# AaronZ345/StyleSinger

Hardware: AMD Instinct MI355X
Metric: mel-frames/sec (end-to-end infer incl. vocoder) (higher is better)
Workload: dtype f32; 1 GPU; c2: batch=8x8.0s utterances per GPU (T=1500 frames, Tp=28, Tr=1500), 100 mel + 2x100 f0 diffusion steps + HiFi-GAN-NSF, exact fp32 MFMA; global_batch=8, frames_per_utterance=1500, parallelism=dp1, diffusion_loops=hipGraph replay, hipgraph_captures=6, frame_bucket=64, mfma_precision=fp32, step_overlap=3 HIP streams: consecutive batches run concurrently

## Files before the change

include/stylesinger_hip.h:

```cpp
#ifndef STYLESINGER_HIP_H
#define STYLESINGER_HIP_H

#include <stdint.h>

#ifdef __cplusplus
extern "C" {
#endif

#define SS_ABI_VERSION 20
#define SS_MAX_TAPS 16
#define SS_MAX_LAYERS 32

const char* ss_last_error(void);
int ss_abi_version(void);
int ss_device_info(int dev, int* n_cu, char* arch, int arch_len);
int ss_struct_sizes(int64_t* out, int n);
int ss_set_tuning(const char* key, int value);
int ss_get_tuning(const char* key);
int ss_set_clock_probe(void* dev_u64x2);
int ss_set_q4_guard(void* dev_u32x2);
int ss_debug_null_launch(int grid, int block, void* stream);

enum {
  SS_EPI_STORE = 0,
  SS_EPI_GATE = 1,
  SS_EPI_RESSKIP = 2,
  SS_EPI_DDPM = 3
};
enum { SS_ACT_NONE_ = 0, SS_ACT_RELU_ = 1, SS_ACT_GELU_ = 2, SS_ACT_MISH_ = 3, SS_ACT_TANH_ = 4, SS_ACT_LRELU_ = 5 };

enum { SS_TILE_AUTO = 0, SS_TILE_128x128 = 1, SS_TILE_64x128 = 2, SS_TILE_64x64 = 3, SS_TILE_128x64 = 4, SS_TILE_128x32 = 5 };

typedef struct ss_conv_gemm_args {
  const float* A;
  int64_t a_batch_stride;
  int32_t lda;
  int32_t Cin;
  int32_t ntaps;
  int32_t tap_off[SS_MAX_TAPS];
  const int32_t* lens;
  int32_t B, T;
  const float* a_bias;
  float a_scale;
  float a_lrelu;
  const float* W;
  int32_t N;
  int32_t Np;
  int32_t Kp;
  int32_t epi;
  const float* bias;
  float pre_scale;
  int32_t act;
  float act_slope;
  const float* E;
  int32_t lde;
  int64_t e_batch_stride;
  int32_t gate_mode;
  const float* R;
  int32_t ldr;
  int64_t r_batch_stride;
  float post_scale;
  int32_t accumulate;
  int32_t mask_rows;
  float* C;
  int32_t ldc;
  int64_t c_batch_stride;
  float* C2;
  int32_t ldc2;
  int64_t c2_batch_stride;
  int32_t Nh;
  float ddpm_recip, ddpm_recipm1, ddpm_c1, ddpm_c2, ddpm_sigma;
  const float* noise;
  uint64_t seed;
  const uint64_t* seed_dev;
  uint32_t step;
  int32_t tile;
  int32_t group_size;
  int64_t w_group_stride, bias_group_stride, a_bias_group_stride;
  int32_t mfma_bf16;
  int32_t ddpm_x0_pred;
  int32_t e_tiled;
  int32_t reserved2_;
} ss_conv_gemm_args;

int ss_conv_gemm(const ss_conv_gemm_args* args, void* stream);

int ss_gemm16_res(const ss_conv_gemm_args* args, int mt, void* stream);
int ss_gemm16_pick(int B, int T, int N);
int ss_gemm16_store(const ss_conv_gemm_args* args, int mt, void* stream);
int ss_gemm16_store_splitk(const ss_conv_gemm_args* args, int mt, int ksplit, float* partials, void* stream);
int ss_gemm16_ksplit_pick(int B, int T, int N, int K);

int ss_gemm16_resw(const ss_conv_gemm_args* args, const float* W16, int mt, void* stream);
int ss_pack_gemm16_weights(const float* src, float* dst, int Np, int Kp, void* stream);
int ss_wino43_gate16w(const ss_conv_gemm_args* args, const float* W16, int dilation, int mt, void* stream);
int ss_pack_gate16_weights(const float* src, float* dst, int Np, int Kp, void* stream);
int ss_wino43_gate16x(const ss_conv_gemm_args* args, const void* Wx, int dilation, int mt, void* stream);
int ss_split3_weights(const float* src, void* dst, int Np, int Kp, void* stream);
int ss_gemm16x_store(const ss_conv_gemm_args* args, const void* Wx, int mt, void* stream);
int ss_split3_gemm16_weights(const float* src, void* dst, int Np, int Kp, void* stream);
int64_t ss_split3_gemm16_elems(int Np, int Kp);
int ss_wino43_conv(const ss_conv_gemm_args* args, int k, int dilation, void* stream);
int ss_wino43_conv_ok(int C, int k, int dilation);
int ss_wino43_conv_ok4(int Cin, int Cout, int k, int dilation);
int ss_wino_gate(const ss_conv_gemm_args* args, int dilation, void* stream);
int ss_wino_weight_transform(const float* src, float* dst, int Cout, int Cin, void* stream);
int ss_wino43_gate(const ss_conv_gemm_args* args, int dilation, void* stream);
int ss_wino43_gate16(const ss_conv_gemm_args* args, int dilation, int mt, void* stream);
int ss_gate16_tile_addend(const float* E, int lde, int64_t e_batch_stride, float* E16, int B, int T, int Np, int dilation, int mt, void* stream);
int64_t ss_gate16_tiled_floats(int B, int T, int Np, int dilation, int mt);
int ss_wino43_gate16_pick(int B, int T, int Np, int dilation);
int ss_wino43_weight_transform(const float* src, float* dst, int Cout, int Cin, void* stream);

enum {
  SS_HEPI_STORE = 0,
  SS_HEPI_GATE = 1,
  SS_HEPI_RESX = 2
};
typedef struct ss_gemm_bf16_args {
  const uint16_t* A;
  int64_t a_batch_stride;
  int32_t lda;
  int32_t K;
  int32_t ntaps;
  int32_t tap_off[4];
  const int32_t* lens;
  int32_t B, T;
  const uint16_t* W;
  int64_t w_group_stride;
  int32_t N, Np;
  int32_t epi;
  int32_t act;
  const float* bias;
  int64_t bias_group_stride;
  const float* E;
  int32_t lde;
  int32_t gate_mode;
  int64_t e_batch_stride;
  float* X;
  int64_t x_batch_stride;
  int32_t ldx;
  float post_scale;
  const float* next_bias;
  int64_t next_bias_group_stride;
  uint16_t* Y;
  int64_t y_batch_stride;
  int32_t ldy;
  int32_t ldc;
  void* C;
  int64_t c_batch_stride;
  int32_t mask_rows;
  int32_t group_size;
  int32_t split;
  float out_scale;
  float q_scale;
  int32_t one_product;
  const float* cur_bias;
  int64_t cur_bias_group_stride;
  int32_t a_compact;
  int32_t reserved2_;
} ss_gemm_bf16_args;
int ss_gemm_bf16(const ss_gemm_bf16_args* args, void* stream);
int ss_gemm_bf16_gate256(const ss_gemm_bf16_args* args, void* stream);
int ss_gemm_bf16_gate256_ok(const ss_gemm_bf16_args* args);
int ss_gemm_bf16_gate128(const ss_gemm_bf16_args* args, void* stream);
int ss_gemm_bf16_gate128_ok(const ss_gemm_bf16_args* args);
int ss_gemm_bf16_gate128q(const ss_gemm_bf16_args* args, void* stream);
int ss_gemm_bf16_gate128q_ok(const ss_gemm_bf16_args* args);
int ss_gate128q_kindex(int32_t* out, int n);
int ss_gemm_bf16_tile256q(const ss_gemm_bf16_args* args, void* stream);
int ss_gemm_bf16_tile256q_ok(const ss_gemm_bf16_args* args);
int ss_tile256q_kindex(int32_t* out, int n_pairs);
int ss_gemm_bf16_tile256(const ss_gemm_bf16_args* args, void* stream);
int ss_gemm_bf16_tile256_ok(const ss_gemm_bf16_args* args);
typedef struct ss_layer512_args {
  const uint16_t* Hin;
  int32_t d;
  int32_t n_products;
  uint16_t* Hout;
  void* P;
  const int32_t* lens;
  int32_t B, T;
  const uint16_t* Wg;
  const uint16_t* Wr;
  const float* E512;
  uint16_t* G;
  int64_t g_batch_stride;
// ... 305 lines not shown
```

stylesinger_amd/csrc/hifigan.hip:

```cpp
#include "common.h"
#include "../../include/stylesinger_hip.h"

namespace {

constexpr int NH = 9;
constexpr int HOP_MAX = 1024;
constexpr size_t LDS_MAX = 160 * 1024;

inline int64_t align_up(int64_t x, int64_t a) { return (x + a - 1) / a * a; }
inline int round_up32(int x) { return (x + 31) / 32 * 32; }

struct HgWs {
  int32_t* lens;
  double* base;
  double* q;
  float* r0;
  float* har;
  float* pre;
  float* x;
  float* xs;
  float* ta;
  float* tb;
  int64_t bytes;
};
// ... 257 lines not shown
__global__ __launch_bounds__(256) void conv_post_kernel(const float* __restrict__ x, const float* __restrict__ w,
                                                        const float* __restrict__ bias, float* __restrict__ wav,
                                                        const int32_t* __restrict__ lens, int B, int64_t L, int C, int k) {
  extern __shared__ float smem[];
  const int ldx = C + 1;
  float* xs = smem;
  float* wsh = smem + (256 + k - 1) * ldx;
  const int tiles = (int)((L + 255) / 256);
  const int b = blockIdx.x / tiles;
  const int64_t i0 = (int64_t)(blockIdx.x % tiles) * 256;
  const int tid = threadIdx.x;
  const int64_t valid = lens ? (int64_t)lens[b] : L;
  const int half = (k - 1) / 2;
  for (int i = tid; i < k * C; i += 256) {
    const int j = i / C, c = i % C;
    wsh[i] = w[c * k + j];
  }
  const int rows = 256 + k - 1;
  for (int i = tid; i < rows * C; i += 256) {
    const int r = i / C, c = i % C;
    const int64_t idx = i0 - half + r;
    float v = 0.f;
    if (idx >= 0 && idx < valid && idx < L) {
      v = x[((int64_t)b * L + idx) * C + c];
      v = v >= 0.f ? v : v * 0.01f;
    }
    xs[r * ldx + c] = v;
  }
  __syncthreads();
  const int64_t i = i0 + tid;
  if (i >= L) return;
  float acc = bias[0];
  for (int j = 0; j < k; ++j)
    for (int c = 0; c < C; ++c) acc += wsh[j * C + c] * xs[(tid + j) * ldx + c];
  wav[(int64_t)b * L + i] = (i < valid) ? tanhf(acc) : 0.f;
}

inline ss_conv_gemm_args base_args(int B, int T, const int32_t* lens) {
  ss_conv_gemm_args a;
  memset(&a, 0, sizeof(a));
  a.B = B;
  a.T = T;
  a.lens = lens;
  a.ntaps = 1;
  a.a_scale = 1.0f;
  a.a_lrelu = 1.0f;
  a.pre_scale = 1.0f;
  a.post_scale = 1.0f;
  a.mask_rows = 1;
  return a;
}

int conv_same(const float* A, int B, int Trows, int C, const int32_t* lens, const float* W, const float* W_wino, const float* bias, int k,
              int d, float lrelu, int act_out, const float* R, float post_scale, int accumulate, float* out, int bf16, hipStream_t stream) {
  ss_conv_gemm_args a = base_args(B, Trows, lens);
  a.mfma_bf16 = bf16;
  a.A = A;
  a.lda = C;
  a.a_batch_stride = (int64_t)Trows * C;
  a.Cin = C;
  a.ntaps = k;
  for (int j = 0; j < k; ++j) a.tap_off[j] = (j - (k - 1) / 2) * d;
  a.a_lrelu = lrelu;
  a.W = W;
  a.N = C;
  a.Np = round_up32(C);
  a.Kp = round_up32(C);
  a.epi = SS_EPI_STORE;
  a.bias = bias;
  a.R = R;
  a.ldr = C;
  a.r_batch_stride = (int64_t)Trows * C;
  a.post_scale = post_scale;
  a.accumulate = accumulate;
  a.C = out;
  a.ldc = C;
  a.c_batch_stride = (int64_t)Trows * C;
  if (act_out) {
    a.act = SS_ACT_LRELU_;
    a.act_slope = 0.1f;
  }
  if (W_wino && ((int64_t)Trows + 1024) * C * 4 < ((int64_t)g_ss_tuning.voc_wino_max_mb << 20)) {
    a.W = W_wino;
    return ss_wino43_conv(&a, k, d, stream);
  }
  return ss_conv_gemm(&a, stream);
}

}

extern "C" int64_t ss_hifigan_workspace_bytes(const ss_hifigan* hg, int B, int T) {
  if (!hg || B <= 0 || T <= 0) return -1;
  return hg_layout(hg, B, T, nullptr).bytes;
}

extern "C" int ss_hifigan_source(const ss_hifigan* hg, const float* f0, int B, int T, const float* rand_ini,
                                 const float* sine_noise, uint64_t seed, float* har, void* ws, int64_t ws_bytes,
                                 void* stream_) {
  hipStream_t stream = (hipStream_t)stream_;
  SS_CHECK_ARG(hg && f0 && har && ws, "ss_hifigan_source: null pointer");
  SS_CHECK_ARG(hg->harmonics + 1 == NH, "ss_hifigan_source: harmonic_num must be 8");
  const int hop = hop_of(hg);
  SS_CHECK_ARG(hop % 64 == 0 && hop <= HOP_MAX, "ss_hifigan_source: hop=%d must be a multiple of 64 and <= %d", hop, HOP_MAX);
  const HgWs w = hg_layout(hg, B, T, ws);
  SS_CHECK_ARG(ws_bytes >= w.bytes, "ss_hifigan_source: workspace too small");
  const float sr = (float)hg->sr;
  hipLaunchKernelGGL(src_base_kernel, dim3(B * NH), dim3(256), 0, stream, f0, rand_ini, seed, w.base, w.r0, B, T, hop, sr);
  SS_CHECK_LAUNCH("src_base_kernel");
  hipLaunchKernelGGL(src_frame_sum_kernel, dim3(B * T), dim3(hop), 0, stream, f0, w.base, w.r0, w.q, B, T, hop, sr);
  SS_CHECK_LAUNCH("src_frame_sum_kernel");
  hipLaunchKernelGGL(src_scan_kernel, dim3(B * NH), dim3(256), 0, stream, w.q, B * NH, T);
  SS_CHECK_LAUNCH("src_scan_kernel");
  hipLaunchKernelGGL(src_final_kernel, dim3(B * T), dim3(hop), 0, stream, f0, w.base, w.r0, w.q, sine_noise, seed,
                     hg->src_w, hg->src_b, har, B, T, hop, sr);
  SS_CHECK_LAUNCH("src_final_kernel");
  return SS_OK;
}

extern "C" int ss_hifigan_forward(const ss_hifigan* hg, const float* mel, const float* f0, const int32_t* lens, int B, int T,
                                  const float* rand_ini, const float* sine_noise, uint64_t seed, float* wav,
                                  float* har_source_out, void* ws, int64_t ws_bytes, void* stream_) {
  hipStream_t stream = (hipStream_t)stream_;
  SS_CHECK_ARG(hg && mel && f0 && wav && ws, "ss_hifigan_forward: null pointer");
  SS_CHECK_ARG(hg->n_ups >= 1 && hg->n_ups <= SS_HG_MAX_UPS && hg->n_kernels >= 1 && hg->n_kernels <= SS_HG_MAX_KERNELS,
               "ss_hifigan_forward: bad config");
  const HgWs w = hg_layout(hg, B, T, ws);
  SS_CHECK_ARG(ws_bytes >= w.bytes, "ss_hifigan_forward: workspace too small (%lld < %lld)", (long long)ws_bytes, (long long)w.bytes);
  const int hop = hop_of(hg);
  const int64_t L = (int64_t)T * hop;

  hipLaunchKernelGGL(stage_lens_kernel, dim3((B + 63) / 64), dim3(64), 0, stream, lens, w.lens, B, T, hg->n_ups,
                     hg->up_rate[0], hg->up_rate[1], hg->up_rate[2], hg->up_rate[3], hg->up_rate[4], hg->up_rate[5]);
  SS_CHECK_LAUNCH("stage_lens_kernel");

  float* har = har_source_out ? har_source_out : w.har;
  SS_PROPAGATE(ss_hifigan_source(hg, f0, B, T, rand_ini, sine_noise, seed, har, ws, ws_bytes, stream_));

  {
    ss_conv_gemm_args a = base_args(B, T, w.lens);
    a.A = mel;
    a.lda = 80;
    a.a_batch_stride = (int64_t)T * 80;
    a.Cin = 80;
    a.ntaps = 7;
    for (int j = 0; j < 7; ++j) a.tap_off[j] = j - 3;
    a.W = hg->w_pre;
    a.N = hg->c0;
    a.Np = round_up32(hg->c0);
    a.Kp = 96;
    a.epi = SS_EPI_STORE;
    a.bias = hg->b_pre;
    a.C = w.pre;
    a.ldc = hg->c0;
    a.c_batch_stride = (int64_t)T * hg->c0;
    a.mfma_bf16 = hg->mfma_bf16;
    SS_PROPAGATE(ss_conv_gemm(&a, stream));
  }

  const float* cur = w.pre;
  int rows_in = T, cin = hg->c0, R = 1;
  for (int i = 0; i < hg->n_ups; ++i) {
    const int u = hg->up_rate[i], ku = hg->up_k[i];
    const int cout = hg->c0 >> (i + 1);
    const int pad = (ku - u) / 2;
    const int nph0 = u - pad;
    const int rows_out = rows_in * u;
// ... 80 lines not shown
```

stylesinger_amd/lib.py:

```python
import ctypes as C
import os

import torch

from . import abi
from .abi import declarations, declared_symbols

HERE = os.path.dirname(os.path.abspath(__file__))
LIB_PATH = os.environ.get("SS_LIB_PATH") or os.path.join(HERE, "libstylesinger_hip.so")

SS_MAX_TAPS, SS_MAX_LAYERS, SS_HG_MAX_UPS, SS_HG_MAX_KERNELS = (abi.DEFINES[n] for n in ("SS_MAX_TAPS", "SS_MAX_LAYERS", "SS_HG_MAX_UPS", "SS_HG_MAX_KERNELS"))
ABI_VERSION = abi.DEFINES["SS_ABI_VERSION"]
ALIGN_MAX_T, ALIGN_MAX_LC = abi.DEFINES["SS_ALIGN_MAX_T"], abi.DEFINES["SS_ALIGN_MAX_LC"]
EPI_STORE, EPI_GATE, EPI_RESSKIP, EPI_DDPM = (abi.ENUMS["SS_EPI_" + n] for n in ("STORE", "GATE", "RESSKIP", "DDPM"))
ACT_NONE, ACT_RELU, ACT_GELU, ACT_MISH, ACT_TANH, ACT_LRELU = (abi.ENUMS[f"SS_ACT_{n}_"] for n in ("NONE", "RELU", "GELU", "MISH", "TANH", "LRELU"))
HEPI_STORE, HEPI_GATE, HEPI_RESX = (abi.ENUMS["SS_HEPI_" + n] for n in ("STORE", "GATE", "RESX"))

_STRUCT_SIZES_ORDER = ("ss_conv_gemm_args", "ss_wavenet", "ss_hifigan", "ss_gemm_bf16_args", "ss_f0track_params", "ss_layer512_args")
ConvGemmArgs, WaveNet, HifiGan, GemmBf16Args, F0TrackParams, Layer512Args = (abi.STRUCTURES[n] for n in _STRUCT_SIZES_ORDER)


class StyleSingerHipError(RuntimeError):
    pass

# ... 93 lines not shown


def gate16_tile_addend(E, *, B, T, Np, lde, e_bs, dilation, mt):
    n = load().ss_gate16_tiled_floats(B, T, Np, int(dilation), int(mt))
    out = torch.empty(n, device=E.device, dtype=torch.float32)
    check(load().ss_gate16_tile_addend(ptr(E), lde, e_bs, ptr(out), B, T, Np, int(dilation), int(mt), stream_ptr()), "ss_gate16_tile_addend")
    return out


def wino_gate(A, Wt, out, *, dilation, **kw):
    kw.setdefault("epi", EPI_GATE)
    a = _fill_args(A, Wt, out, **kw)
    check(load().ss_wino_gate(C.byref(a), int(dilation), stream_ptr()), "ss_wino_gate")


def wino43_gate(A, Wt, out, *, dilation, **kw):
    kw.setdefault("epi", EPI_GATE)
    a = _fill_args(A, Wt, out, **kw)
    check(load().ss_wino43_gate(C.byref(a), int(dilation), stream_ptr()), "ss_wino43_gate")


def pack_gemm16_weights(Wp, Kp):
    Wp = Wp.contiguous().float()
    out = torch.empty_like(Wp)
    check(load().ss_pack_gemm16_weights(ptr(Wp), ptr(out), Wp.shape[0], Kp, stream_ptr()), "ss_pack_gemm16_weights")
    return out


def pack_gate16_weights(Wp, Kp):
    Wp = Wp.contiguous().float()
    out = torch.empty_like(Wp)
    check(load().ss_pack_gate16_weights(ptr(Wp), ptr(out), Wp.shape[0], Kp, stream_ptr()), "ss_pack_gate16_weights")
    return out


def wino43_gate16(A, Wt, out, *, dilation, mt=0, W16=None, **kw):
    kw.setdefault("epi", EPI_GATE)
    a = _fill_args(A, Wt, out, **kw)
    if W16 is not None:
        check(load().ss_wino43_gate16w(C.byref(a), ptr(W16), int(dilation), int(mt), stream_ptr()), "ss_wino43_gate16w")
        return
    check(load().ss_wino43_gate16(C.byref(a), int(dilation), int(mt), stream_ptr()), "ss_wino43_gate16")


def gemm16_res(A, W, out, *, mt=0, W16=None, **kw):
    a = _fill_args(A, W, out, **kw)
    if W16 is not None:
        check(load().ss_gemm16_resw(C.byref(a), ptr(W16), int(mt), stream_ptr()), "ss_gemm16_resw")
        return
    check(load().ss_gemm16_res(C.byref(a), int(mt), stream_ptr()), "ss_gemm16_res")


def gemm16_store(A, W, out, *, mt=0, **kw):
    a = _fill_args(A, W, out, **kw)
    check(load().ss_gemm16_store(C.byref(a), int(mt), stream_ptr()), "ss_gemm16_store")


def gemm16_store_splitk(A, W, out, *, ksplit, mt=0, **kw):
    a = _fill_args(A, W, out, **kw)
    part = torch.empty(max(1, ksplit) * a.B * a.T * a.N, device=out.device, dtype=torch.float32)
    check(load().ss_gemm16_store_splitk(C.byref(a), int(mt), int(ksplit), ptr(part), stream_ptr()), "ss_gemm16_store_splitk")


def wino43_weight(w):
    w = w.contiguous().float()
    out = torch.empty(w.shape[0], w.shape[1], 6, device=w.device, dtype=torch.float32)
    check(load().ss_wino43_weight_transform(ptr(w), ptr(out), w.shape[0], w.shape[1], stream_ptr()), "ss_wino43_weight_transform")
    return out


def wino43_group_weight(w):
    w = w.contiguous().float()
    Cout, Cin, k = w.shape
    G = (k + 2) // 3
    wp = torch.zeros(Cout, Cin, 3 * G, device=w.device, dtype=torch.float32)
    wp[..., :k] = w
    return torch.cat([wino43_weight(wp[..., 3 * g:3 * g + 3]) for g in range(G)], dim=-1).contiguous()


def wino43_conv(A, W, out, *, k, dilation, **kw):
    taps = [(j - (k - 1) // 2) * dilation for j in range(k)]
    a = _fill_args(A, W, out, taps=taps, **kw)
    check(load().ss_wino43_conv(C.byref(a), k, dilation, stream_ptr()), "ss_wino43_conv")
    return out


def split3_weights(Wp, Kp):
    Wp = Wp.contiguous().float()
    Np = Wp.shape[0]
    out = torch.empty(Np, 3 * Wp.shape[1], device=Wp.device, dtype=torch.bfloat16)
    check(load().ss_split3_weights(ptr(Wp), ptr(out), Np, Kp, stream_ptr()), "ss_split3_weights")
    return out


def split3_gemm16_weights(Wp, Kp):
    Wp = Wp.contiguous().float()
    Np = Wp.shape[0]
    out = torch.empty(int(load().ss_split3_gemm16_elems(Np, Kp)), device=Wp.device, dtype=torch.bfloat16)
    check(load().ss_split3_gemm16_weights(ptr(Wp), ptr(out), Np, Kp, stream_ptr()), "ss_split3_gemm16_weights")
    return out


def gemm16x_store(A, W, Wx, out, *, mt=0, **kw):
    a = _fill_args(A, W, out, **kw)
    check(load().ss_gemm16x_store(C.byref(a), ptr(Wx), int(mt), stream_ptr()), "ss_gemm16x_store")


def wino43_gate16x(A, Wx, out, *, dilation, mt=0, **kw):
    kw.setdefault("epi", EPI_GATE)
    a = _fill_args(A, Wx, out, **kw)
    check(load().ss_wino43_gate16x(C.byref(a), ptr(Wx), dilation, mt, stream_ptr()), "ss_wino43_gate16x")
    return out


def wino_weight(w):
    w = w.contiguous().float()
    out = torch.empty(w.shape[0], w.shape[1], 4, device=w.device, dtype=torch.float32)
    check(load().ss_wino_weight_transform(ptr(w), ptr(out), w.shape[0], w.shape[1], stream_ptr()), "ss_wino_weight_transform")
    return out


def pack_conv_weight(w, *, scale0=None, interleave_half=0, row_scale=1.0):
    if w.dim() == 2:
        w = w[:, :, None]
    w = w.contiguous().float()
    Cout, Cin, k = w.shape
    Kp = round_up(Cin, 32)
    Np = 2 * round_up(interleave_half, 32) if interleave_half else round_up(Cout, 32)
    dst = torch.empty(Np, k * Kp, device=w.device, dtype=torch.float32)
    check(load().ss_pack_conv_weight(ptr(w), ptr(scale0), ptr(dst), Cout, Cin, k, Np, Kp, interleave_half, _f(row_scale),
                                     stream_ptr()), "ss_pack_conv_weight")
    return dst


def weight_norm_scale(v, g):
    v = v.contiguous().float()
    g = g.contiguous().float().reshape(-1)
    rows = v.shape[0]
    out = torch.empty(rows, device=v.device, dtype=torch.float32)
    check(load().ss_weight_norm_scale(ptr(v), ptr(g), ptr(out), rows, v.numel() // rows, stream_ptr()), "ss_weight_norm_scale")
    return out


def pack_convtr_weight(w, scale0, u, group):
    w = w.contiguous().float()
    Cin, Cout, k = w.shape
    pad = (k - u) // 2
    nph = (u - pad) if group == 0 else pad
    Np = round_up(nph * Cout, 32)
    Kp = round_up(Cin, 32)
    dst = torch.empty(Np, 2 * Kp, device=w.device, dtype=torch.float32)
    check(load().ss_pack_convtr_weight(ptr(w), ptr(scale0), ptr(dst), Cin, Cout, k, u, group, Np, Kp, stream_ptr()),
          "ss_pack_convtr_weight")
    return dst


def pack_bias(b, *, b2=None, Np=None, interleave_half=0, repeat=1):
    b = b.contiguous().float()
    n = b.numel()
    if Np is None:
        Np = 2 * round_up(interleave_half, 32) if interleave_half else round_up(n * repeat, 32)
    dst = torch.empty(Np, device=b.device, dtype=torch.float32)
    check(load().ss_pack_bias(ptr(b), ptr(b2), ptr(dst), n, Np, interleave_half, repeat, stream_ptr()), "ss_pack_bias")
    return dst


# ... 275 lines not shown
```

stylesinger_amd/vocoder.py:

```python
import ctypes

import numpy as np
import torch

from . import lib as L
from . import spec as _spec
from .config import make_hparams, make_vocoder_config
from .denoise import denoise_batch, geometry as denoise_geometry, resolve_denoise

REGISTERED_VOCODERS = {}


def register_vocoder(name):
    def _f(cls):
        REGISTERED_VOCODERS[name] = cls
        return cls
    return _f


def get_vocoder_cls(hparams):
    return REGISTERED_VOCODERS[hparams["vocoder"]]


CONV_POST_MAX_CHANNELS = 128
# ... 34 lines not shown
        bad("upsample_initial_channel", f"must halve {len(rates)} times into a multiple of 4 channels")
    if c0 >> len(rates) > CONV_POST_MAX_CHANNELS:
        bad("upsample_initial_channel", f"leaves {c0 >> len(rates)} channels for conv_post, at most {CONV_POST_MAX_CHANNELS}")
    rk, rd = cfg.get("resblock_kernel_sizes"), cfg.get("resblock_dilation_sizes")
    if not ints(rk) or not 1 <= len(rk) <= L.SS_HG_MAX_KERNELS:
        bad("resblock_kernel_sizes", f"1 to {L.SS_HG_MAX_KERNELS} integer kernel sizes")
    for k in rk:
        if k < 1 or k % 2 == 0 or k > L.SS_MAX_TAPS:
            bad("resblock_kernel_sizes", f"kernel {k}: odd and at most {L.SS_MAX_TAPS} taps")
    if not isinstance(rd, (list, tuple)) or len(rd) != len(rk):
        bad("resblock_dilation_sizes", "one list of dilations per ResBlock kernel size")
    for d in rd:
        if not ints(d) or len(d) != 3 or min(d) < 1:
            bad("resblock_dilation_sizes", f"{list(d) if isinstance(d, (list, tuple)) else d!r}: exactly three positive dilations per ResBlock")
    return cfg


class HifiGanGeneratorHIP(torch.nn.Module):

    def __init__(self, h=None):
        super().__init__()
        self.h = make_vocoder_config(h)
        self._names = []
        for name, shape in _spec.vocoder_spec(self.h):
            self._names.append(name)
            self.register_buffer("p__" + name.replace(".", "__"), torch.zeros(*shape))
        self._pk = None
        self._weights_version = 0
        self._packed_version = -1
        self.hop = int(np.prod(self.h["upsample_rates"]))

    def p(self, name):
        return getattr(self, "p__" + name.replace(".", "__"))

    def state_dict(self, *a, **k):
        return {n: self.p(n) for n in self._names}

    def load_state_dict(self, state_dict, strict=True):
        missing = [n for n in self._names if n not in state_dict]
        unexpected = [k for k in state_dict if k not in set(self._names)]
        if strict and (missing or unexpected):
            raise RuntimeError(f"HifiGanGeneratorHIP.load_state_dict: missing={missing[:5]} unexpected={unexpected[:5]}")
        with torch.no_grad():
            for n in self._names:
                if n in state_dict:
                    self.p(n).copy_(state_dict[n])
        self._weights_version += 1
        return torch.nn.modules.module._IncompatibleKeys(missing, unexpected)

    def remove_weight_norm(self):
        return self

    def _wn(self, prefix):
        v, g = self.p(prefix + ".weight_v"), self.p(prefix + ".weight_g")
        return v, L.weight_norm_scale(v, g)

    def pack(self):
        h = check_config(self.h)
        dev = self.p("conv_pre.bias").device
        if dev.type != "cuda":
            raise L.StyleSingerHipError("HifiGanGeneratorHIP needs its weights on a GPU: there is no CPU path")
        keep = []
        hg = L.HifiGan()
        rates, ks = h["upsample_rates"], h["upsample_kernel_sizes"]
        hg.n_ups, hg.n_kernels, hg.c0 = len(rates), len(h["resblock_kernel_sizes"]), h["upsample_initial_channel"]
        hg.sr, hg.harmonics = h["audio_sample_rate"], h["harmonic_num"]
        import os
        hg.mfma_bf16 = 1 if os.environ.get("SS_PRECISION", h.get("mfma_precision", "fp32")) == "bf16" else 0
        hg.wino = 1 if (not hg.mfma_bf16 and os.environ.get("SS_VOC_WINO", str(h.get("vocoder_wino", 1))) != "0") else 0
        lib = L.load()
        for i, (u, k) in enumerate(zip(rates, ks)):
            hg.up_rate[i], hg.up_k[i] = u, k
        for i in range(len(rates), L.SS_HG_MAX_UPS):
            hg.up_rate[i], hg.up_k[i] = 1, 1
        for j, k in enumerate(h["resblock_kernel_sizes"]):
            hg.rb_k[j] = k
            for m, d in enumerate(h["resblock_dilation_sizes"][j]):
                hg.rb_d[j][m] = d

        def hold(t):
            keep.append(t)
            return t.data_ptr()

        v, s0 = self._wn("conv_pre")
        hg.w_pre = hold(L.pack_conv_weight(v, scale0=s0))
        hg.b_pre = hold(L.pack_bias(self.p("conv_pre.bias")))
        nk = hg.n_kernels
        for i, u in enumerate(rates):
            v, s0 = self._wn(f"ups.{i}")
            for g in range(2):
                hg.w_up[i][g] = hold(L.pack_convtr_weight(v, s0, u, g))
            hg.b_up[i] = hold(L.pack_bias(self.p(f"ups.{i}.bias"), repeat=u))
            hg.w_noise[i] = hold(self.p(f"noise_convs.{i}.weight").contiguous())
            hg.b_noise[i] = hold(self.p(f"noise_convs.{i}.bias").contiguous())
            for j in range(nk):
                for m in range(3):
                    pfx = f"resblocks.{i * nk + j}"
                    k, d = h["resblock_kernel_sizes"][j], h["resblock_dilation_sizes"][j][m]
                    cout = hg.c0 >> (i + 1)
                    v, s0 = self._wn(f"{pfx}.convs1.{m}")
                    hg.w_rb1[i][j][m] = hold(L.pack_conv_weight(v, scale0=s0))
                    hg.b_rb1[i][j][m] = hold(L.pack_bias(self.p(f"{pfx}.convs1.{m}.bias")))
                    if hg.wino and lib.ss_wino43_conv_ok(cout, k, d):
                        hg.w_rb1_wino[i][j][m] = hold(L.pack_conv_weight(L.wino43_group_weight(v * s0.view(-1, 1, 1))))
                    v, s0 = self._wn(f"{pfx}.convs2.{m}")
                    hg.w_rb2[i][j][m] = hold(L.pack_conv_weight(v, scale0=s0))
                    hg.b_rb2[i][j][m] = hold(L.pack_bias(self.p(f"{pfx}.convs2.{m}.bias")))
                    if hg.wino and lib.ss_wino43_conv_ok(cout, k, 1):
                        hg.w_rb2_wino[i][j][m] = hold(L.pack_conv_weight(L.wino43_group_weight(v * s0.view(-1, 1, 1))))
        v, s0 = self._wn("conv_post")
        hg.w_post = hold((v * s0.view(-1, 1, 1)).contiguous())
        hg.b_post = hold(self.p("conv_post.bias").contiguous())
        hg.src_w = hold(self.p("m_source.l_linear.weight").reshape(-1).contiguous())
        hg.src_b = hold(self.p("m_source.l_linear.bias").contiguous())
        self._pk = dict(hg=hg, keep=keep)
        self._packed_version = self._weights_version
        self._pack_device = dev
        torch.cuda.synchronize()

    def _ensure_packed(self):
        dev = self.p("conv_pre.bias").device
        if self._pk is None or self._packed_version != self._weights_version or self._pack_device != dev:
            self.pack()

    @torch.no_grad()
    def forward(self, mel, f0, lens=None, noise=None, seed=1234, return_source=False):
        self._ensure_packed()
        lib = L.load()
        hg = self._pk["hg"]
        mel = mel.contiguous().float()
        f0 = f0.contiguous().float()
        B, T, _ = mel.shape
        dev = mel.device
        Ls = T * self.hop
        wav = torch.empty(B, Ls, device=dev, dtype=torch.float32)
        har = torch.empty(B, Ls, device=dev, dtype=torch.float32) if return_source else None
        ws_bytes = lib.ss_hifigan_workspace_bytes(ctypes.addressof(hg), B, T)
        ws = torch.empty(ws_bytes, device=dev, dtype=torch.uint8)
        ri = sn = None
        if noise is not None:
            ri = noise["rand_ini"].to(dev).contiguous().float()
            sn = noise["sine_noise"].to(dev).contiguous().float()
        L.check(lib.ss_hifigan_forward(ctypes.addressof(hg), L.ptr(mel), L.ptr(f0), L.ptr(lens), B, T, L.ptr(ri), L.ptr(sn), seed,
                                       L.ptr(wav), L.ptr(har), L.ptr(ws), ws_bytes, L.stream_ptr()), "ss_hifigan_forward")
        return (wav, har) if return_source else wav


class BaseVocoder:
    def spec2wav(self, mel, **kwargs):
        raise NotImplementedError


@register_vocoder("HifiGAN_NSF")
class HifiGAN(BaseVocoder):

    def __init__(self, config=None, state_dict=None, device="cuda", hparams=None):
        self.hparams = make_hparams(hparams)
        self._denoise_v = resolve_denoise(self.hparams)
        self.config = make_vocoder_config(config)
        self.device = torch.device(device)
        self.model = HifiGanGeneratorHIP(self.config)
        if state_dict is not None:
            self.model.load_state_dict(state_dict, strict=True)
        self.model.remove_weight_norm()
        self.model.eval().to(self.device)

    def spec2wav(self, mel, **kwargs):
        f0 = kwargs.get("f0")
        if f0 is None or not self.hparams.get("use_nsf", True):
            raise NotImplementedError("the HIP vocoder implements the NSF path (use_nsf: true, f0 given)")
        c = torch.as_tensor(np.asarray(mel), dtype=torch.float32)[None].to(self.device)
        f = torch.as_tensor(np.asarray(f0), dtype=torch.float32)[None].to(self.device)
        y = self.model(c, f, noise=kwargs.get("noise"), seed=kwargs.get("seed", 1234))
        if self._denoise_v is not None:
            n_fft, hop = denoise_geometry(self.hparams)
            y, _ = denoise_batch(y, [y.shape[1]], n_fft, hop, n_fft, self._denoise_v)
        return y.view(-1).cpu().numpy()

    def spec2wav_batch(self, mel, f0, lens=None, **kwargs):
        out = self.model(mel, f0, lens=lens, **kwargs)
        if self._denoise_v is None:
            return out
        n_fft, hop = denoise_geometry(self.hparams)
        if hop != self.model.hop:
            raise L.StyleSingerHipError(f"vocoder_denoise_c: hop_size={hop} is not supported on the batched path: must equal the generator's hop "
                                        f"({self.model.hop})")
        wav = out[0] if isinstance(out, tuple) else out
        wav, _ = denoise_batch(wav, None if lens is None else lens * hop, n_fft, hop, n_fft, self._denoise_v)
        return (wav,) + tuple(out[1:]) if isinstance(out, tuple) else wav
```

Baseline: 44280 mel-frames/s.

## Add Winograd F(4,4) conv kernel for vocoder resblocks with k=7/11

Adds a new Winograd F(4,4) 1D convolution kernel using 7 transformed points per group of 4 taps. The vocoder resblock convs dispatch to it whenever it needs fewer MFMA products than the existing F(4,3) path, which is the case for kernel sizes 7 and 11. The goal is to cut the multiply work in the HiFi-GAN resblocks. In exchange it uses larger input-transform coefficients (up to 5 and 32/45), which can cost fp32 accuracy, and it brings a new pipelined kernel with its own LDS double-buffering.

```diff
diff --git a/include/stylesinger_hip.h b/include/stylesinger_hip.h
--- a/include/stylesinger_hip.h
+++ b/include/stylesinger_hip.h
@@ -103,6 +103,8 @@
 int ss_wino43_conv(const ss_conv_gemm_args* args, int k, int dilation, void* stream);
 int ss_wino43_conv_ok(int C, int k, int dilation);
 int ss_wino43_conv_ok4(int Cin, int Cout, int k, int dilation);
+int ss_wino44_conv(const ss_conv_gemm_args* args, int k, int dilation, void* stream);
+int ss_wino44_conv_ok(int C, int k, int dilation);
 int ss_wino_gate(const ss_conv_gemm_args* args, int dilation, void* stream);
 int ss_wino_weight_transform(const float* src, float* dst, int Cout, int Cin, void* stream);
 int ss_wino43_gate(const ss_conv_gemm_args* args, int dilation, void* stream);
diff --git a/stylesinger_amd/csrc/hifigan.hip b/stylesinger_amd/csrc/hifigan.hip
--- a/stylesinger_amd/csrc/hifigan.hip
+++ b/stylesinger_amd/csrc/hifigan.hip
@@ -363,6 +363,7 @@
   }
   if (W_wino && ((int64_t)Trows + 1024) * C * 4 < ((int64_t)g_ss_tuning.voc_wino_max_mb << 20)) {
     a.W = W_wino;
+    if (ss_wino44_conv_ok(C, k, d)) return ss_wino44_conv(&a, k, d, stream);
     return ss_wino43_conv(&a, k, d, stream);
   }
   return ss_conv_gemm(&a, stream);
diff --git a/stylesinger_amd/csrc/wino44_conv.hip b/stylesinger_amd/csrc/wino44_conv.hip
--- /dev/null
+++ b/stylesinger_amd/csrc/wino44_conv.hip
@@ -0,0 +1,373 @@
+#include "common.h"
+#include "device_prims.h"
+#include "../../include/stylesinger_hip.h"
+#include <type_traits>
+
+namespace {
+
+using namespace ss_dev;
+
+constexpr int BK = 32;
+constexpr int LD = BK;
+constexpr int BQ = 64;
+constexpr int NC = 7;
+constexpr int NR = 7;
+
+template <int D>
+__device__ __forceinline__ int frame_of_quad(int q) {
+  if constexpr (D == 1) return 4 * q;
+  else return (q / D) * (4 * D) + (q % D);
+}
+
+template <int D, bool LRELU, int BN>
+__global__ __launch_bounds__(BN * 4, BN == 64 ? 2 : 1) void wino44_conv_kernel(const ss_conv_gemm_args a, int q_tiles_per_item, int q_tiles,
+                                                                               int n_tiles, int groups, int lo_rows) {
+  static_assert(BN == 64 || BN == 32, "column tile of 64 or 32");
+  constexpr int NT = BN * 4;
+  constexpr int RP = NT / 8;
+  constexpr int AP = BQ / RP;
+  constexpr int BP = BN / RP;
+  extern __shared__ __attribute__((aligned(16))) float smem[];
+  float* As = smem;
+  float* Bs = smem + 2 * BQ * LD;
+
+  const int id = blockIdx.x;
+  const int grp = id / (8 * n_tiles);
+  const int rem = id % (8 * n_tiles);
+  const int qt = grp * 8 + (rem & 7);
+  const int nt = rem >> 3;
+  if (qt >= q_tiles) return;
+  const int b = __builtin_amdgcn_readfirstlane(qt / q_tiles_per_item);
+  const int q0 = __builtin_amdgcn_readfirstlane((qt % q_tiles_per_item) * BQ);
+  const int n0 = nt * BN;
+
+  const int tid = threadIdx.x, lane = tid & 63, wave = tid >> 6;
+  const int wm = BN == 64 ? wave >> 1 : wave, wn = BN == 64 ? wave & 1 : 0;
+  const int l31 = lane & 31, lh = lane >> 5;
+
+  const int len = ss_uniform_len(a.lens, b, a.T);
+  const int kchunks = a.Kp / BK;
+  const int ldw = groups * NC * a.Kp;
+
+  const __amdgpu_buffer_rsrc_t rsrc_a = __builtin_amdgcn_make_buffer_rsrc(
+      uniform_ptr(a.A + (int64_t)b * a.a_batch_stride), 0, __builtin_amdgcn_readfirstlane(len * a.lda * 4), 0x00020000);
+  const __amdgpu_buffer_rsrc_t rsrc_w =
+      __builtin_amdgcn_make_buffer_rsrc(uniform_ptr(a.W), 0, __builtin_amdgcn_readfirstlane(a.Np * ldw * 4), 0x00020000);
+
+  const int st_c4 = tid & 7;
+  const int st_row = tid >> 3;
+  int roff[AP];
+#pragma unroll
+  for (int i = 0; i < AP; ++i) roff[i] = ((frame_of_quad<D>(q0 + st_row + i * RP) - lo_rows) * a.lda + st_c4 * 4) * 4;
+  const int row_step = D * a.lda * 4;
+  const int group_step = 4 * row_step;
+  int w_voff[BP];
+#pragma unroll
+  for (int i = 0; i < BP; ++i) w_voff[i] = ((n0 + st_row + i * RP) * ldw + st_c4 * 4) * 4;
+
+  using Yes = std::true_type;
+  using No = std::false_type;
+  u32x4 rr[AP][NR], rb[BP];
+  auto load_rows = [&](int ci0b, auto ends) {
+    ci0b = __builtin_amdgcn_readfirstlane(ci0b);
+#pragma unroll
+    for (int i = 0; i < AP; ++i)
+#pragma unroll
+      for (int r = 0; r < NR; ++r)
+        if ((r == 0 || r == NR - 1) == decltype(ends)::value) rr[i][r] = __builtin_amdgcn_raw_buffer_load_b128(rsrc_a, roff[i] + r * row_step, ci0b, 0);
+  };
+  auto load_b = [&](int cb) {
+    cb = __builtin_amdgcn_readfirstlane(cb);
+#pragma unroll
+    for (int i = 0; i < BP; ++i) rb[i] = __builtin_amdgcn_raw_buffer_load_b128(rsrc_w, w_voff[i], cb, 0);
+  };
+  const float slope = a.a_lrelu;
+  auto act_rows = [&]() {
+    if constexpr (LRELU) {
+#pragma unroll
+      for (int i = 0; i < AP; ++i)
+#pragma unroll
+        for (int r = 0; r < NR; ++r) {
+          const f32x4 v = __builtin_bit_cast(f32x4, rr[i][r]);
+          const f32x4 sv = v * slope;
+          f32x4 o;
+          o.x = ss_lrelu_max(v.x, sv.x);
+          o.y = ss_lrelu_max(v.y, sv.y);
+          o.z = ss_lrelu_max(v.z, sv.z);
+          o.w = ss_lrelu_max(v.w, sv.w);
+          rr[i][r] = __builtin_bit_cast(u32x4, o);
+        }
+    }
+  };
+  int a_wr[AP];
+#pragma unroll
+  for (int i = 0; i < AP; ++i) a_wr[i] = lds_slot(st_row + i * RP, st_c4);
+  float4 tU[AP], tV[AP], tW[AP];
+  auto store_a = [&](float* Ad, auto ptag) {
+    constexpr int P = decltype(ptag)::value;
+#pragma unroll
+    for (int i = 0; i < AP; ++i) {
+      auto R = [&](int q) { return __builtin_bit_cast(float4, rr[i][q]); };
+      float4 v;
+      if constexpr (P == 0) {
+        tU[i] = vfma(4.f, R(1), vfma(-5.f, R(3), R(5)));
+        tV[i] = vfma(4.f, R(0), vfma(-5.f, R(2), R(4)));
+        tW[i] = vfma(4.f, R(2), vfma(-5.f, R(4), R(6)));
+        v = tU[i];
+      } else if constexpr (P == 1) {
+        v = vfma(-0.5f, tU[i], tW[i]);
+      } else if constexpr (P == 2) {
+        v = vfma(-0.5f, tV[i], tU[i]);
+      } else if constexpr (P == 3) {
+        tV[i] = vfma(2.f, R(1), vfma(-4.f, R(2), vfma(-0.5f, R(3), R(4))));
+        tU[i] = vfma(2.f, R(2), vfma(-4.f, R(3), vfma(-0.5f, R(4), R(5))));
+        v = vadd(tU[i], tV[i]);
+      } else if constexpr (P == 4) {
+        v = vsub(tU[i], tV[i]);
+      } else if constexpr (P == 5) {
+        tV[i] = vfma(0.5f, R(1), vfma(-0.5f, R(3), vsub(R(4), R(2))));
+        tU[i] = vfma(0.5f, R(2), vfma(-0.5f, R(4), vsub(R(5), R(3))));
+        v = vfma(2.f, tV[i], tU[i]);
+      } else {
+        v = vfma(-2.f, tV[i], tU[i]);
+      }
+      *reinterpret_cast<float4*>(Ad + a_wr[i]) = v;
+    }
+  };
+  auto store_b = [&](float* Bd) {
+#pragma unroll
+    for (int i = 0; i < BP; ++i)
+      *reinterpret_cast<float4*>(Bd + lds_slot(st_row + i * RP, st_c4)) = __builtin_bit_cast(float4, rb[i]);
+  };
+
+  f32x16 acc[NC];
+#pragma unroll
+  for (int j = 0; j < NC; ++j)
+#pragma unroll
+    for (int r = 0; r < 16; ++r) acc[j][r] = 0.f;
+
+  constexpr int ORD[NC] = {5, 6, 0, 1, 2, 3, 4};
+  const int kb = a.Kp * 4;
+  const int cs = BK * 4;
+  const int steps = groups * kchunks;
+
+  const int swz = (l31 >> 1) & 7;
+  const int a_row = (wm * 32 + l31) * LD;
+  const int b_row = (wn * 32 + l31) * LD;
+  auto read_frags = [&](const float* Ac, const float* Bc, int q, float4& af, float4& bf) {
+    const int so = ((2 * q + lh) ^ swz) << 2;
+    af = *reinterpret_cast<const float4*>(Ac + a_row + so);
+    bf = *reinterpret_cast<const float4*>(Bc + b_row + so);
+  };
+  auto mfma4 = [&](f32x16& c, const float4& af, const float4& bf) {
+    c = __builtin_amdgcn_mfma_f32_32x32x2f32(af.x, bf.x, c, 0, 0, 0);
+    c = __builtin_amdgcn_mfma_f32_32x32x2f32(af.y, bf.y, c, 0, 0, 0);
+    c = __builtin_amdgcn_mfma_f32_32x32x2f32(af.z, bf.z, c, 0, 0, 0);
+    c = __builtin_amdgcn_mfma_f32_32x32x2f32(af.w, bf.w, c, 0, 0, 0);
+  };
+  auto chunk = [&](auto etag, auto ptag, auto stage_tag, auto fetch_b_tag, auto fetch_rows_tag, int wb, int rows_cb, bool new_group) {
+    constexpr int P = decltype(ptag)::value;
+    constexpr int CUR = (decltype(etag)::value + P) & 1;
+    constexpr int PN = (P + 1) % NC;
+    const float* Ac = As + CUR * BQ * LD;
+    const float* Bc = Bs + CUR * BN * LD;
+    float4 af0, af1, bf0, bf1;
+    read_frags(Ac, Bc, 0, af0, bf0);
+    read_frags(Ac, Bc, 1, af1, bf1);
+    __builtin_amdgcn_sched_barrier(0);
+    mfma4(acc[ORD[P]], af0, bf0);
+    read_frags(Ac, Bc, 2, af0, bf0);
+    __builtin_amdgcn_sched_barrier(0);
+    mfma4(acc[ORD[P]], af1, bf1);
+    read_frags(Ac, Bc, 3, af1, bf1);
+    __builtin_amdgcn_sched_barrier(0);
+    if constexpr (decltype(stage_tag)::value) {
+      if constexpr (PN == 0) act_rows();
+      store_a(As + (CUR ^ 1) * BQ * LD, std::integral_constant<int, PN>{});
+      store_b(Bs + (CUR ^ 1) * BN * LD);
+    }
+    __builtin_amdgcn_sched_barrier(0);
+    if constexpr (decltype(fetch_b_tag)::value) load_b(wb);
+    if constexpr (decltype(fetch_rows_tag)::value) {
+      if constexpr (P == 4) {
+        if (new_group) {
+#pragma unroll
+          for (int i = 0; i < AP; ++i) roff[i] += group_step;
+        }
+        load_rows(rows_cb, No{});
+      } else {
+        load_rows(rows_cb, Yes{});
+      }
+    }
+    __builtin_amdgcn_sched_barrier(0);
+    mfma4(acc[ORD[P]], af0, bf0);
+    mfma4(acc[ORD[P]], af1, bf1);
+    __syncthreads();
+  };
+  using P0 = std::integral_constant<int, 0>;
+  using P1 = std::integral_constant<int, 1>;
+  using P2 = std::integral_constant<int, 2>;
+  using P3 = std::integral_constant<int, 3>;
+  using P4 = std::integral_constant<int, 4>;
+  using P5 = std::integral_constant<int, 5>;
+  using P6 = std::integral_constant<int, 6>;
+
+  int g = 0, k = 0;
+  auto step = [&](auto etag) {
+    const bool wrap = k + 1 == kchunks;
+    const int gn = wrap ? g + 1 : g, kn = wrap ? 0 : k + 1;
+    const int wcur = g * NC * kb + k * cs, wnext = gn * NC * kb + kn * cs;
+    chunk(etag, P0{}, Yes{}, Yes{}, No{}, wcur + ORD[2] * kb, 0, false);
+    chunk(etag, P1{}, Yes{}, Yes{}, No{}, wcur + ORD[3] * kb, 0, false);
+    chunk(etag, P2{}, Yes{}, Yes{}, No{}, wcur + ORD[4] * kb, 0, false);
+    chunk(etag, P3{}, Yes{}, Yes{}, No{}, wcur + ORD[5] * kb, 0, false);
+    chunk(etag, P4{}, Yes{}, Yes{}, Yes{}, wcur + ORD[6] * kb, kn * cs, wrap);
+    chunk(etag, P5{}, Yes{}, Yes{}, Yes{}, wnext + ORD[0] * kb, kn * cs, false);
+    chunk(etag, P6{}, Yes{}, Yes{}, No{}, wnext + ORD[1] * kb, 0, false);
+    g = gn;
+    k = kn;
+  };
+  using E0 = std::integral_constant<int, 0>;
+  using E1 = std::integral_constant<int, 1>;
+
+  load_rows(0, No{});
+  load_rows(0, Yes{});
+  load_b(ORD[0] * kb);
+  act_rows();
+  store_a(As, P0{});
+  store_b(Bs);
+  load_b(ORD[1] * kb);
+  __syncthreads();
+
+  auto last_step = [&](auto etag) {
+    const int wcur = g * NC * kb + k * cs;
+    chunk(etag, P0{}, Yes{}, Yes{}, No{}, wcur + ORD[2] * kb, 0, false);
+    chunk(etag, P1{}, Yes{}, Yes{}, No{}, wcur + ORD[3] * kb, 0, false);
+    chunk(etag, P2{}, Yes{}, Yes{}, No{}, wcur + ORD[4] * kb, 0, false);
+    chunk(etag, P3{}, Yes{}, Yes{}, No{}, wcur + ORD[5] * kb, 0, false);
+    chunk(etag, P4{}, Yes{}, Yes{}, No{}, wcur + ORD[6] * kb, 0, false);
+    chunk(etag, P5{}, Yes{}, No{}, No{}, 0, 0, false);
+    chunk(etag, P6{}, No{}, No{}, No{}, 0, 0, false);
+  };
+  if constexpr (BN == 64) {
+    for (int s = 0; s + 2 < steps; s += 2) {
+      step(E0{});
+      step(E1{});
+    }
+    step(E0{});
+    last_step(E1{});
+  } else {
+    int left = steps;
+    for (; left > 2; left -= 2) {
+      step(E0{});
+      step(E1{});
+    }
+    if (left == 2) {
+      step(E0{});
+      last_step(E1{});
+    } else {
+      last_step(E0{});
+    }
+  }
+
+  const int col = n0 + wn * 32 + l31;
+  const bool col_ok = col < a.N;
+  const int oob = col_ok ? 0 : (int)0x80000000;
+  const __amdgpu_buffer_rsrc_t rsrc_c = __builtin_amdgcn_make_buffer_rsrc(
+      uniform_ptr(a.C + (int64_t)b * a.c_batch_stride), 0, __builtin_amdgcn_readfirstlane((int)((int64_t)a.T * a.ldc * 4)), 0x00020000);
+  const __amdgpu_buffer_rsrc_t rsrc_r = __builtin_amdgcn_make_buffer_rsrc(
+      uniform_ptr(a.R ? const_cast<float*>(a.R) + (int64_t)b * a.r_batch_stride : a.C), 0,
+      __builtin_amdgcn_readfirstlane(a.R ? (int)((int64_t)a.T * a.ldr * 4) : 0), 0x00020000);
+  const __amdgpu_buffer_rsrc_t rsrc_p = __builtin_amdgcn_make_buffer_rsrc(
+      uniform_ptr(a.C + (int64_t)b * a.c_batch_stride), 0, __builtin_amdgcn_readfirstlane(a.accumulate ? (int)((int64_t)a.T * a.ldc * 4) : 0),
+      0x00020000);
+  const float bs = (a.bias && col_ok) ? a.bias[col] : 0.f;
+  const int row_lim = a.mask_rows ? (len < a.T ? len : a.T) : a.T;
+  const int ldc4 = a.ldc * 4, ldr4 = a.ldr * 4;
+  const int qbase = q0 + wm * 32 + 4 * lh;
+  const bool lrelu_out = a.act == SS_ACT_LRELU_;
+#pragma unroll
+  for (int rb4 = 0; rb4 < 4; ++rb4) {
+    float rv[4][4], pv[4][4];
+    int tq[4];
+#pragma unroll
+    for (int e = 0; e < 4; ++e) {
+      tq[e] = frame_of_quad<D>(qbase + e + 8 * rb4);
+#pragma unroll
+      for (int o = 0; o < 4; ++o) {
+        const int t = tq[e] + o * D;
+        rv[e][o] = __builtin_bit_cast(float, __builtin_amdgcn_raw_buffer_load_b32(rsrc_r, t * ldr4 + (col * 4 + oob), 0, 0));
+        pv[e][o] = __builtin_bit_cast(float, __builtin_amdgcn_raw_buffer_load_b32(rsrc_p, t * ldc4 + (col * 4 + oob), 0, 0));
+      }
+    }
+#pragma unroll
+    for (int e = 0; e < 4; ++e) {
+      const int r = e + 4 * rb4;
+      const float s12 = acc[1][r] + acc[2][r], d12 = acc[1][r] - acc[2][r];
+      const float s34 = acc[3][r] + acc[4][r], d34 = acc[3][r] - acc[4][r];
+      const float m5 = acc[5][r];
+      float z[4];
+      z[0] = (acc[0][r] + s12) + (s34 + m5);
+      z[1] = fmaf(0.5f, m5, fmaf(2.0f, d34, d12));
+      z[2] = fmaf(0.25f, m5, fmaf(4.0f, s34, s12));
+      z[3] = fmaf(0.125f, m5, fmaf(8.0f, d34, d12)) + acc[6][r];
+#pragma unroll
+      for (int o = 0; o < 4; ++o) {
+        const int t = tq[e] + o * D;
+        float v = (z[o] + bs) * a.pre_scale;
+        if (lrelu_out) v = ss_lrelu(v, a.act_slope);
+        v = (v + rv[e][o]) * a.post_scale + pv[e][o];
+        if (t >= row_lim) v = 0.f;
+        __builtin_amdgcn_raw_buffer_store_b32(__builtin_bit_cast(unsigned, v), rsrc_c, t * ldc4 + (col * 4 + oob), 0, 0);
+      }
+    }
+  }
+}
+
+template <int D, int BN>
+void launch_conv(const ss_conv_gemm_args& a, int k, hipStream_t stream) {
+  const int quads_per_item = ss_cdiv(a.T, 4 * D) * D;
+  const int q_tiles_per_item = ss_cdiv(quads_per_item, BQ);
+  const int q_tiles = q_tiles_per_item * a.B;
+  const int n_tiles = a.Np / BN;
+  const int grid = ss_cdiv(q_tiles, 8) * 8 * n_tiles;
+  const size_t lds = (size_t)2 * (BQ + BN) * LD * sizeof(float);
+  const int groups = (k + 3) / 4, lo = (k - 1) / 2 * D;
+  auto go = [&](auto kernel) { hipLaunchKernelGGL(kernel, dim3(grid), dim3(BN * 4), lds, stream, a, q_tiles_per_item, q_tiles, n_tiles, groups, lo); };
+  if (a.a_lrelu != 1.0f) go(wino44_conv_kernel<D, true, BN>);
+  else go(wino44_conv_kernel<D, false, BN>);
+}
+
+template <int D>
+void launch_conv(const ss_conv_gemm_args& a, int k, hipStream_t stream) {
+  if (a.Np % 64 == 0) launch_conv<D, 64>(a, k, stream);
+  else launch_conv<D, 32>(a, k, stream);
+}
+
+}
+
+extern "C" int ss_wino44_conv_ok(int C, int k, int dilation) {
+  const bool fewer = k >= 1 && k <= 11 && (k & 1) && ((k + 3) / 4) * 7 < ((k + 2) / 3) * 6;
+  return fewer && C > 0 && C % 32 == 0 && (dilation == 1 || dilation == 3 || dilation == 5) ? 1 : 0;
+}
+
+extern "C" int ss_wino44_conv(const ss_conv_gemm_args* args, int k, int dilation, void* stream) {
+  SS_CHECK_ARG(args != nullptr, "ss_wino44_conv: null args");
+  const ss_conv_gemm_args& a = *args;
+  SS_CHECK_ARG(a.A && a.W && a.C, "ss_wino44_conv: null A/W/C");
+  SS_CHECK_ARG(a.Cin == a.N && ss_wino44_conv_ok(a.Cin, k, dilation), "ss_wino44_conv: Cin=%d == N=%d (multiple of 32), k=%d (7|11), dilation=%d (1|3|5)",
+               a.Cin, a.N, k, dilation);
+  SS_CHECK_ARG(a.Kp == a.Cin && a.Np == a.N && (a.lda & 3) == 0 && a.lda >= a.Cin, "ss_wino44_conv: Kp == Cin, Np == N, lda a multiple of 4");
+  SS_CHECK_ARG(a.epi == SS_EPI_STORE && (a.act == SS_ACT_NONE_ || a.act == SS_ACT_LRELU_) && !a.a_bias && a.a_scale == 1.0f && !a.mfma_bf16 &&
+                   a.group_size == 0,
+               "ss_wino44_conv: STORE epilogue, act none|lrelu, no input bias/scale, fp32, one weight set");
+  SS_CHECK_ARG(a.a_lrelu > 0.0f && a.a_lrelu <= 1.0f, "ss_wino44_conv: input leaky-relu slope %g must be in (0, 1]", (double)a.a_lrelu);
+  SS_CHECK_ARG(((int64_t)a.T + 1024) * a.lda * 4 < (1ll << 31) && (int64_t)a.T * a.ldc * 4 < (1ll << 31) &&
+                   (!a.R || (int64_t)a.T * a.ldr * 4 < (1ll << 31)) && (int64_t)a.Np * ((k + 3) / 4) * NC * a.Kp * 4 < (1ll << 31),
+               "ss_wino44_conv: item too large for 32-bit offsets");
+  if (dilation == 1) launch_conv<1>(a, k, (hipStream_t)stream);
+  else if (dilation == 3) launch_conv<3>(a, k, (hipStream_t)stream);
+  else launch_conv<5>(a, k, (hipStream_t)stream);
+  SS_CHECK_LAUNCH("ss_wino44_conv");
+  return SS_OK;
+}
diff --git a/stylesinger_amd/lib.py b/stylesinger_amd/lib.py
--- a/stylesinger_amd/lib.py
+++ b/stylesinger_amd/lib.py
@@ -199,6 +199,37 @@
     taps = [(j - (k - 1) // 2) * dilation for j in range(k)]
     a = _fill_args(A, W, out, taps=taps, **kw)
     check(load().ss_wino43_conv(C.byref(a), k, dilation, stream_ptr()), "ss_wino43_conv")
+    return out
+
+
+WINO44_G = (
+    (-1 / 2, 0.0, 0.0, 0.0),
+    (-1 / 3, -1 / 3, -1 / 3, -1 / 3),
+    (1 / 9, -1 / 9, 1 / 9, -1 / 9),
+    (1 / 36, 1 / 18, 1 / 9, 2 / 9),
+    (-1 / 60, 1 / 30, -1 / 15, 2 / 15),
+    (32 / 45, 16 / 45, 8 / 45, 4 / 45),
+    (0.0, 0.0, 0.0, 1.0),
+)
+
+
+def wino44_conv_ok(C, k, dilation):
+    return int(load().ss_wino44_conv_ok(int(C), int(k), int(dilation)))
+
+
+def wino44_group_weight(w):
+    Cout, Cin, k = w.shape
+    G = (k + 3) // 4
+    wp = torch.zeros(Cout, Cin, G, 4, device=w.device, dtype=torch.float64)
+    wp.view(Cout, Cin, 4 * G)[..., :k] = w.double()
+    g = torch.tensor(WINO44_G, device=w.device, dtype=torch.float64)
+    return torch.einsum("jt,oigt->oigj", g, wp).reshape(Cout, Cin, 7 * G).float().contiguous()
+
+
+def wino44_conv(A, W, out, *, k, dilation, **kw):
+    taps = [(j - (k - 1) // 2) * dilation for j in range(k)]
+    a = _fill_args(A, W, out, taps=taps, **kw)
+    check(load().ss_wino44_conv(C.byref(a), k, dilation, stream_ptr()), "ss_wino44_conv")
     return out
 
 
diff --git a/stylesinger_amd/vocoder.py b/stylesinger_amd/vocoder.py
--- a/stylesinger_amd/vocoder.py
+++ b/stylesinger_amd/vocoder.py
@@ -140,6 +140,9 @@
             keep.append(t)
             return t.data_ptr()
 
+        def wino_group(c, k, d):
+            return L.wino44_group_weight if L.wino44_conv_ok(c, k, d) else L.wino43_group_weight
+
         v, s0 = self._wn("conv_pre")
         hg.w_pre = hold(L.pack_conv_weight(v, scale0=s0))
         hg.b_pre = hold(L.pack_bias(self.p("conv_pre.bias")))
@@ -160,12 +163,12 @@
                     hg.w_rb1[i][j][m] = hold(L.pack_conv_weight(v, scale0=s0))
                     hg.b_rb1[i][j][m] = hold(L.pack_bias(self.p(f"{pfx}.convs1.{m}.bias")))
                     if hg.wino and lib.ss_wino43_conv_ok(cout, k, d):
-                        hg.w_rb1_wino[i][j][m] = hold(L.pack_conv_weight(L.wino43_group_weight(v * s0.view(-1, 1, 1))))
+                        hg.w_rb1_wino[i][j][m] = hold(L.pack_conv_weight(wino_group(cout, k, d)(v * s0.view(-1, 1, 1))))
                     v, s0 = self._wn(f"{pfx}.convs2.{m}")
                     hg.w_rb2[i][j][m] = hold(L.pack_conv_weight(v, scale0=s0))
                     hg.b_rb2[i][j][m] = hold(L.pack_bias(self.p(f"{pfx}.convs2.{m}.bias")))
                     if hg.wino and lib.ss_wino43_conv_ok(cout, k, 1):
-                        hg.w_rb2_wino[i][j][m] = hold(L.pack_conv_weight(L.wino43_group_weight(v * s0.view(-1, 1, 1))))
+                        hg.w_rb2_wino[i][j][m] = hold(L.pack_conv_weight(wino_group(cout, k, 1)(v * s0.view(-1, 1, 1))))
         v, s0 = self._wn("conv_post")
         hg.w_post = hold((v * s0.view(-1, 1, 1)).contiguous())
         hg.b_post = hold(self.p("conv_post.bias").contiguous())
```

Result: faster. 44890 mel-frames/s, median of 6 (+1.4%).
